# russellgeum/Digging-into-Self-Supervised-Monocular-Depth-Estimation

Hardware: AMD Instinct MI355X
Metric: images/sec training, KITTI 192x640 batch 12/GPU (higher is better)
Workload: dtype f32; 1 GPU; configs[1]: kitti_eigen_zhou-shaped 192x640, batch 12/GPU, ResNet18 depth + separate ResNet18 pose, frame_ids [0,-1,1], 4 scales, automask, Adam, fp32; global_batch=12, parallelism=dp1

## Files before the change

digging-into-self-supervised-monocular-depth-estimation_amd/csrc/norm_nhwc.hip:

```cpp
#include "nhwc_common.hpp"

namespace mdx {
namespace nhwc {

constexpr int STATS_FWD_BLOCKS = 256;
constexpr int STATS_BWD_BLOCKS_F32 = 256, STATS_BWD_BLOCKS_BF16 = 384;
constexpr int STATS_MAX_BLOCKS = 384;
constexpr int APPLY_MAX_BLOCKS = 4096;
constexpr int STATS_ITERS = 8, APPLY_ITERS = 4;
static inline int stats_bwd_blocks(int dtype) { return dtype == 0 ? STATS_BWD_BLOCKS_F32 : STATS_BWD_BLOCKS_BF16; }

template <typename T>
__global__ __launch_bounds__(NB) void bn_nhwc_fwd_stats_kernel(const T *__restrict__ x, int M, int C, int CVB, int PL, int RB,
                                                               float *__restrict__ part)
{
    constexpr int N = VecN<T>::N;
    __shared__ float lds[2 * NB * N];
    const Pos p = position<N>(M, C, CVB, PL, RB);
    float a[N], q[N];
#pragma unroll
    for (int j = 0; j < N; ++j) a[j] = q[j] = 0.f;
    if (p.active) {
        const T *px = x + (size_t)p.g * M * C + (size_t)p.cv * N;
        auto acc = [&](const Vec<T, N> &v) {
// ... 137 lines not shown
    for (; r + 3 * PL < p.r1; r += 4 * PL) {
        const size_t o0 = (size_t)r * C, o1 = (size_t)(r + PL) * C, o2 = (size_t)(r + 2 * PL) * C, o3 = (size_t)(r + 3 * PL) * C;
        const Vec<T, N> v0 = load_vec<T, N>(px + o0), v1 = load_vec<T, N>(px + o1), v2 = load_vec<T, N>(px + o2), v3 = load_vec<T, N>(px + o3);
        Vec<T, N> r0 = {}, r1 = {}, r2 = {}, r3 = {};
        if (pr) { r0 = load_vec<T, N>(pr + o0); r1 = load_vec<T, N>(pr + o1); r2 = load_vec<T, N>(pr + o2); r3 = load_vec<T, N>(pr + o3); }
        apply(v0, r0, o0); apply(v1, r1, o1); apply(v2, r2, o2); apply(v3, r3, o3);
    }
    for (; r < p.r1; r += PL) {
        const size_t o = (size_t)r * C;
        Vec<T, N> rv = {};
        if (pr) rv = load_vec<T, N>(pr + o);
        apply(load_vec<T, N>(px + o), rv, o);
    }
}

template <typename T, bool MASKX>
__global__ __launch_bounds__(NB) void bn_nhwc_bwd_stats_kernel(const T *__restrict__ dy, const T *__restrict__ dy2,
                                                               const T *__restrict__ y, const T *__restrict__ x,
                                                               const float *__restrict__ gamma, const float *__restrict__ beta,
                                                               const float *__restrict__ save_mean,
                                                               const float *__restrict__ save_invstd, int M, int C, int CVB, int PL,
                                                               int RB, int relu, float *__restrict__ part)
{
    constexpr int N = VecN<T>::N;
    __shared__ float lds[2 * NB * N];
    const Pos p = position<N>(M, C, CVB, PL, RB);
    float a[N], q[N];
#pragma unroll
    for (int j = 0; j < N; ++j) a[j] = q[j] = 0.f;
    if (p.active) {
        float mean[N], invstd[N], scale[N], shift[N];
#pragma unroll
        for (int j = 0; j < N; ++j) {
            mean[j] = save_mean[(size_t)p.g * C + p.cv * N + j];
            invstd[j] = save_invstd[(size_t)p.g * C + p.cv * N + j];
            scale[j] = shift[j] = 0.f;
            if (MASKX) {
                scale[j] = gamma[p.cv * N + j] * invstd[j];
                shift[j] = beta[p.cv * N + j] - mean[j] * scale[j];
            }
        }
        const size_t base = (size_t)p.g * M * C + (size_t)p.cv * N;
        const T *pd = dy + base, *pd2 = dy2 ? dy2 + base : nullptr, *py = MASKX ? nullptr : y + base, *px = x + base;
        auto acc = [&](const Vec<T, N> &vd, const Vec<T, N> &vd2, const Vec<T, N> &vy, const Vec<T, N> &vx) {
#pragma unroll
            for (int j = 0; j < N; ++j) {
                float d = to_float(vd.v[j]);
                if (pd2) d += to_float(vd2.v[j]);
                const float yv = !MASKX ? to_float(vy.v[j]) : to_float(from_float<T>(__builtin_fmaf(to_float(vx.v[j]), scale[j], shift[j])));
                const float dz = (relu && !(yv > 0.f)) ? 0.f : d;
                a[j] += dz;
                q[j] = __builtin_fmaf(dz, (to_float(vx.v[j]) - mean[j]) * invstd[j], q[j]);
            }
        };
        int r = p.r0 + p.pl;
        for (; r + PL < p.r1; r += 2 * PL) {
            const size_t o0 = (size_t)r * C, o1 = (size_t)(r + PL) * C;
            const Vec<T, N> d0 = load_vec<T, N>(pd + o0), d1 = load_vec<T, N>(pd + o1);
            Vec<T, N> y0 = {}, y1 = {};
            if (!MASKX) { y0 = load_vec<T, N>(py + o0); y1 = load_vec<T, N>(py + o1); }
            const Vec<T, N> x0 = load_vec<T, N>(px + o0), x1 = load_vec<T, N>(px + o1);
            Vec<T, N> e0 = {}, e1 = {};
            if (pd2) { e0 = load_vec<T, N>(pd2 + o0); e1 = load_vec<T, N>(pd2 + o1); }
            acc(d0, e0, y0, x0);
            acc(d1, e1, y1, x1);
        }
        for (; r < p.r1; r += PL) {
            const size_t o = (size_t)r * C;
            Vec<T, N> e = {}, yv = {};
            if (pd2) e = load_vec<T, N>(pd2 + o);
            if (!MASKX) yv = load_vec<T, N>(py + o);
            acc(load_vec<T, N>(pd + o), e, yv, load_vec<T, N>(px + o));
        }
    }
    block_partials<N>(a, q, lds, CVB, PL, C, part + ((size_t)p.g * gridDim.x + blockIdx.x) * 2 * C);
}

template <typename T, bool MASKX>
__global__ __launch_bounds__(NB) void bn_nhwc_bwd_apply_kernel(const T *__restrict__ dy, const T *__restrict__ dy2,
                                                               const T *__restrict__ y, const T *__restrict__ x,
                                                               const float *__restrict__ gamma, const float *__restrict__ beta,
                                                               const float *__restrict__ save_mean,
                                                               const float *__restrict__ save_invstd,
                                                               const float *__restrict__ totals, int M, int C, int CVB, int PL,
                                                               int RB, int relu, T *__restrict__ dx, T *__restrict__ dres)
{
    constexpr int N = VecN<T>::N;
    const Pos p = position<N>(M, C, CVB, PL, RB);
    if (!p.active) return;
    float mean[N], invstd[N], k0[N], mdz[N], mdzx[N], shift[N];
#pragma unroll
    for (int j = 0; j < N; ++j) {
        const int c = p.cv * N + j;
        mean[j] = save_mean[(size_t)p.g * C + c];
        invstd[j] = save_invstd[(size_t)p.g * C + c];
        k0[j] = gamma[c] * invstd[j];
        shift[j] = MASKX ? beta[c] - mean[j] * k0[j] : 0.f;
        mdz[j] = totals[((size_t)p.g * 2 + 0) * C + c];
        mdzx[j] = totals[((size_t)p.g * 2 + 1) * C + c];
    }
    const size_t base = (size_t)p.g * M * C + (size_t)p.cv * N;
    const T *pd = dy + base, *pd2 = dy2 ? dy2 + base : nullptr, *py = MASKX ? nullptr : y + base, *px = x + base;
    T *ox = dx + base;
    T *orr = dres ? dres + base : nullptr;
    auto apply = [&](const Vec<T, N> &vd, const Vec<T, N> &vd2, const Vec<T, N> &vy, const Vec<T, N> &vx, size_t off) {
        Vec<T, N> wx, wr;
#pragma unroll
        for (int j = 0; j < N; ++j) {
            float d = to_float(vd.v[j]);
            if (pd2) d += to_float(vd2.v[j]);
            const float yv = !MASKX ? to_float(vy.v[j]) : to_float(from_float<T>(__builtin_fmaf(to_float(vx.v[j]), k0[j], shift[j])));
            const float dz = (relu && !(yv > 0.f)) ? 0.f : d;
            const float xh = (to_float(vx.v[j]) - mean[j]) * invstd[j];
            wx.v[j] = from_float<T>(k0[j] * (dz - mdz[j] - xh * mdzx[j]));
            wr.v[j] = from_float<T>(dz);
        }
        store_vec<T, N>(ox + off, wx);
        if (orr) store_vec<T, N>(orr + off, wr);
    };
    int r = p.r0 + p.pl;
    for (; r + PL < p.r1; r += 2 * PL) {
        const size_t o0 = (size_t)r * C, o1 = (size_t)(r + PL) * C;
        const Vec<T, N> d0 = load_vec<T, N>(pd + o0), d1 = load_vec<T, N>(pd + o1);
        Vec<T, N> y0 = {}, y1 = {};
        if (!MASKX) { y0 = load_vec<T, N>(py + o0); y1 = load_vec<T, N>(py + o1); }
        const Vec<T, N> x0 = load_vec<T, N>(px + o0), x1 = load_vec<T, N>(px + o1);
        Vec<T, N> e0 = {}, e1 = {};
        if (pd2) { e0 = load_vec<T, N>(pd2 + o0); e1 = load_vec<T, N>(pd2 + o1); }
        apply(d0, e0, y0, x0, o0);
        apply(d1, e1, y1, x1, o1);
    }
    for (; r < p.r1; r += PL) {
        const size_t o = (size_t)r * C;
        Vec<T, N> e = {}, yv = {};
        if (pd2) e = load_vec<T, N>(pd2 + o);
        if (!MASKX) yv = load_vec<T, N>(py + o);
        apply(load_vec<T, N>(pd + o), e, yv, load_vec<T, N>(px + o), o);
    }
}

static inline int vec_elems(int dtype) { return dtype == 0 ? 4 : 8; }

}
}

using namespace mdx;
using namespace mdx::nhwc;

MDX_EXPORT size_t mdx_bn_nhwc_workspace_bytes(int B, int C, int H, int W, int groups, int dtype)
{
    if (B <= 0 || C <= 0 || H <= 0 || W <= 0 || groups <= 0 || (dtype != 0 && dtype != 1)) return 0;
    const Rows g = make_rows((long long)B * H * W, C, vec_elems(dtype), STATS_MAX_BLOCKS, STATS_ITERS);
// ... 52 lines not shown
    if (bad) return bad;
    if (!aligned(dy, 16) || (y && !aligned(y, 16)) || !aligned(x, 16) || !aligned(dx, 16) || (dy2 && !aligned(dy2, 16)) ||
        (dres && !aligned(dres, 16)))
        return MDX_ERR_MISALIGNED;
    if (workspace_bytes < mdx_bn_nhwc_workspace_bytes(B, C, H, W, groups, dtype)) return MDX_ERR_WORKSPACE;
    const int M = B * H * W, N = vec_elems(dtype);
    const Rows gs = make_rows(M, C, N, stats_bwd_blocks(dtype), STATS_ITERS), ga = make_rows(M, C, N, APPLY_MAX_BLOCKS, APPLY_ITERS);
    float *part = (float *)workspace;
    float *totals = part + (size_t)groups * gs.nblk * 2 * C;
    hipStream_t st = (hipStream_t)stream;
    const dim3 grid_s(gs.nblk, gs.t.ny, groups), grid_a(ga.nblk, ga.t.ny, groups), block(NB);
    const bool maskx = !y;
#define MDX_BN_BWD(KERNEL, T, MX, ...) hipLaunchKernelGGL((KERNEL<T, MX>), __VA_ARGS__)
    if (dtype == 0 && maskx)
        MDX_BN_BWD(bn_nhwc_bwd_stats_kernel, float, true, grid_s, block, 0, st, (const float *)dy, (const float *)dy2, (const float *)y,
                   (const float *)x, gamma, beta, save_mean, save_invstd, M, C, gs.t.CVB, gs.t.PL, gs.RB, relu, part);
    else if (dtype == 0)
        MDX_BN_BWD(bn_nhwc_bwd_stats_kernel, float, false, grid_s, block, 0, st, (const float *)dy, (const float *)dy2, (const float *)y,
                   (const float *)x, gamma, beta, save_mean, save_invstd, M, C, gs.t.CVB, gs.t.PL, gs.RB, relu, part);
    else if (maskx)
        MDX_BN_BWD(bn_nhwc_bwd_stats_kernel, bf16, true, grid_s, block, 0, st, (const bf16 *)dy, (const bf16 *)dy2, (const bf16 *)y,
                   (const bf16 *)x, gamma, beta, save_mean, save_invstd, M, C, gs.t.CVB, gs.t.PL, gs.RB, relu, part);
    else
        MDX_BN_BWD(bn_nhwc_bwd_stats_kernel, bf16, false, grid_s, block, 0, st, (const bf16 *)dy, (const bf16 *)dy2, (const bf16 *)y,
                   (const bf16 *)x, gamma, beta, save_mean, save_invstd, M, C, gs.t.CVB, gs.t.PL, gs.RB, relu, part);
    hipLaunchKernelGGL(bn_nhwc_bwd_finalize_kernel, dim3((C + FC - 1) / FC), dim3(FC * FS), 0, st, part, gs.nblk, C, groups, (double)M, totals,
                       dgamma, dbeta);
    if (dtype == 0 && maskx)
        MDX_BN_BWD(bn_nhwc_bwd_apply_kernel, float, true, grid_a, block, 0, st, (const float *)dy, (const float *)dy2, (const float *)y,
                   (const float *)x, gamma, beta, save_mean, save_invstd, totals, M, C, ga.t.CVB, ga.t.PL, ga.RB, relu, (float *)dx, (float *)dres);
    else if (dtype == 0)
        MDX_BN_BWD(bn_nhwc_bwd_apply_kernel, float, false, grid_a, block, 0, st, (const float *)dy, (const float *)dy2, (const float *)y,
                   (const float *)x, gamma, beta, save_mean, save_invstd, totals, M, C, ga.t.CVB, ga.t.PL, ga.RB, relu, (float *)dx, (float *)dres);
    else if (maskx)
        MDX_BN_BWD(bn_nhwc_bwd_apply_kernel, bf16, true, grid_a, block, 0, st, (const bf16 *)dy, (const bf16 *)dy2, (const bf16 *)y,
                   (const bf16 *)x, gamma, beta, save_mean, save_invstd, totals, M, C, ga.t.CVB, ga.t.PL, ga.RB, relu, (bf16 *)dx, (bf16 *)dres);
    else
        MDX_BN_BWD(bn_nhwc_bwd_apply_kernel, bf16, false, grid_a, block, 0, st, (const bf16 *)dy, (const bf16 *)dy2, (const bf16 *)y,
                   (const bf16 *)x, gamma, beta, save_mean, save_invstd, totals, M, C, ga.t.CVB, ga.t.PL, ga.RB, relu, (bf16 *)dx, (bf16 *)dres);
#undef MDX_BN_BWD
    return check_launch();
}
```

digging-into-self-supervised-monocular-depth-estimation_amd/mdx/functional.py:

```python
import ctypes as C

import torch

from . import _lib
from ._lib import api, ptr, stream


def _f32c(t):
    return t.contiguous().float() if (t.dtype != torch.float32 or not t.is_contiguous()) else t


def _ws(nbytes, device):
    return torch.empty(max(int(nbytes), 8) // 8 + 1, dtype=torch.float64, device=device)


class _ComposeProjection(torch.autograd.Function):
    @staticmethod
    def forward(ctx, K, T):
        K, T = _f32c(K), _f32c(T)
        B = K.shape[0]
        P = torch.empty(B, 3, 4, device=K.device, dtype=torch.float32)
        api.mdx_compose_projection(ptr(K), ptr(T), B, ptr(P), stream())
        ctx.save_for_backward(K, T)
        return P
# ... 976 lines not shown
            nws = api.mdx_bn_workspace_bytes(Bg, Cc, H, W)
            ws = torch.empty(nws // 4 + 1, device=x.device, dtype=torch.float32)
            api.mdx_bn_act_bwd(
                ptr(dy, x.dtype), ptr(y, x.dtype), ptr(x, x.dtype), ptr(weight), ptr(save_mean), ptr(save_invstd),
                ptr(dx, x.dtype), ptr(dres, x.dtype) if has_res else None, ptr(dgamma), ptr(dbeta), Bg, Cc, H, W, groups,
                int(relu), code, ptr(ws), nws, stream())
        return (dx, dres, dgamma, dbeta) + (None,) * 7


def bn_act(x, weight, bias, running_mean, running_var, eps=1e-5, momentum=0.1, residual=None, relu=True, groups=1,
           fork=False):
    return _BnAct.apply(x, residual, weight, bias, running_mean, running_var, float(eps), float(momentum), bool(relu),
                        int(groups), bool(fork))


def bn_act_infer(x, weight, bias, running_mean, running_var, eps=1e-5, residual=None, relu=True, fork=False):
    code = _glue_dtype(x, "bn_act_infer")
    B, Cc, H, W = x.shape
    cl = is_channels_last(x) and _nhwc_ok(x.dtype, Cc)
    x = _as(x, cl)
    if residual is not None:
        if residual.shape != x.shape or residual.dtype != x.dtype:
            raise _lib.MdxError("bn_act_infer: residual %s %s does not match x %s %s"
                                % (tuple(residual.shape), residual.dtype, tuple(x.shape), x.dtype))
        residual = _as(residual, cl)
    y = torch.empty_like(x)
    fn = api.mdx_bn_act_nhwc_infer if cl else api.mdx_bn_act_infer
    fn(ptr(x, x.dtype, cl=cl), ptr(residual, x.dtype, cl=cl) if residual is not None else None, ptr(_f32c(weight)),
       ptr(_f32c(bias)), ptr(_f32c(running_mean)), ptr(_f32c(running_var)), ptr(y, x.dtype, cl=cl), B, Cc, H, W, float(eps),
       int(bool(relu)), code, stream())
# ... 78 lines not shown
```

digging-into-self-supervised-monocular-depth-estimation_amd/model_layer/depth_encoder.py:

```python
import os
import warnings

import numpy as np
import torch
import torch.nn as nn
import torch.nn.functional as TF



class BatchNorm2d(nn.BatchNorm2d):

    fused_min_elements = 0
    fused_eval = True
    _batch_groups = 1

    @staticmethod
    def batch_groups(groups, network):
        import contextlib

        @contextlib.contextmanager
        def scope():
            mods = [m for m in network.modules() if isinstance(m, BatchNorm2d)]
            prev = [m.__dict__.get("_batch_groups") for m in mods]
            for m in mods:
# ... 21 lines not shown
        return self._norm(x)

    def _norm(self, x):
        if self.training:
            self._pending_batches += 1
        return TF.batch_norm(x, self.running_mean, self.running_var, self.weight, self.bias, self.training,
                             self.momentum, self.eps)

    def act(self, x, residual=None, relu=True, fork=False):
        if not self.training and self._eval_fused(x, residual):
            from mdx import functional as F
            if residual is not None and residual.dtype != x.dtype:
                residual = residual.to(x.dtype)
            return F.bn_act_infer(x, self.weight, self.bias, self.running_mean, self.running_var, self.eps,
                                  residual=residual, relu=relu, fork=fork)
        fused = (self.training and x.is_cuda and self.track_running_stats and self.momentum is not None
                 and self.affine and x.dtype in (torch.float32, torch.bfloat16) and x.dim() == 4
                 and torch.is_grad_enabled() and x.shape[0] % self._batch_groups == 0
                 and x.shape[0] * x.shape[2] * x.shape[3] >= self.fused_min_elements
                 and (x.shape[0] // self._batch_groups) * ((x.shape[2] * x.shape[3] + 8191) // 8192) <= 65535)
        if not fused:
            out = self(x)
            if residual is not None:
                out = out + residual
            out = TF.relu(out) if relu else out
            return (out, out) if fork else out
        from mdx import functional as F
        self._pending_batches += self._batch_groups
        if residual is not None and residual.dtype != x.dtype:
            residual = residual.to(x.dtype)
        return F.bn_act(x, self.weight, self.bias, self.running_mean, self.running_var, self.eps, self.momentum,
                        residual=residual, relu=relu, groups=self._batch_groups, fork=fork)

    def _eval_fused(self, x, residual):
        if not (self.fused_eval and x.is_cuda and x.dtype in (torch.float32, torch.bfloat16) and x.dim() == 4
                and self.track_running_stats and self.affine and self.running_mean is not None):
            return False
        return not torch.is_grad_enabled() or not any(
            t is not None and t.requires_grad for t in (x, residual, self.weight, self.bias))

    def _flush_counter(self):
        if self._pending_batches and self.num_batches_tracked is not None:
            self.num_batches_tracked += self._pending_batches
        self._pending_batches = 0

    def _save_to_state_dict(self, destination, prefix, keep_vars):
        self._flush_counter()
        super()._save_to_state_dict(destination, prefix, keep_vars)

    def _load_from_state_dict(self, *args, **kwargs):
        self._pending_batches = 0
        super()._load_from_state_dict(*args, **kwargs)

def _pair(x):
    return x if isinstance(x, tuple) else (x, x)


class BasicBlock(nn.Module):
    expansion = 1
    fork_output = True

    def __init__(self, inplanes, planes, stride=1, downsample=None):
        super().__init__()
        self.conv1 = nn.Conv2d(inplanes, planes, 3, stride, 1, bias=False)
        self.bn1 = BatchNorm2d(planes)
        self.relu = nn.ReLU(inplace=True)
        self.conv2 = nn.Conv2d(planes, planes, 3, 1, 1, bias=False)
# ... 94 lines not shown
        super().__init__()
        self.num_ch_enc = np.array([64, 64, 128, 256, 512])
        if num_layers not in _CFG:
            raise ValueError("{} is not a valid number of resnet layers".format(num_layers))
        if num_input_images > 1:
            self.encoder = resnet_multiimage_input(num_layers, pretrained, num_input_images)
        else:
            block, layers = _CFG[num_layers]
            self.encoder = ResNet(block, layers)
            if pretrained:
                _load_pretrained(self.encoder, num_layers, 1)
        if num_layers > 34:
            self.num_ch_enc[1:] *= 4

    fused_input = True

    def _normalised_input(self, input_image):
        from mdx import functional as F
        from mdx.layout import weight_layout
        stack = input_image if isinstance(input_image, F.FrameStack) else None
        if stack is None and torch.is_tensor(input_image) and input_image.dim() == 4 and input_image.shape[1] == 3:
            stack = F.FrameStack([[input_image]])
        if (self.fused_input and stack is not None and stack.ok() and weight_layout(self.encoder.conv1)
                and stack.blocks[0][0].numel() * len(stack.blocks) * len(stack.blocks[0]) < (1 << 31)):
            dt = torch.get_autocast_gpu_dtype() if torch.is_autocast_enabled() else torch.float32
            if dt in (torch.float32, torch.bfloat16):
                return F.encoder_input(stack, 0.45, 0.225, dt)
        if isinstance(input_image, F.FrameStack):
            input_image = input_image.tensor()
        return (input_image - 0.45) / 0.225

    def forward(self, input_image):
        from mdx.layout import to_layout, weight_layout
        self.features = []
        x = self._normalised_input(input_image)
        stem, stem_b = _pair(self.encoder.bn1.act(self.encoder.conv1(x), fork=BasicBlock.fork_output))
        self.features.append(stem)
        if (stem.is_cuda and stem.dtype in (torch.float32, torch.bfloat16)
                and stem.shape[0] * stem.shape[1] <= 65535):
            from mdx import functional as F
            x = F.maxpool3s2(stem_b, fork=BasicBlock.fork_output)
        else:
            x = self.encoder.maxpool(stem_b)
        for layer in (self.encoder.layer1, self.encoder.layer2, self.encoder.layer3, self.encoder.layer4):
            x = _pair(layer(to_layout(x, weight_layout(layer)) if x[0].is_cuda else x))
            self.features.append(x[0])
        return self.features
```

digging-into-self-supervised-monocular-depth-estimation_amd/model_tool/loader.py:

```python
import os

import torch
from torch.utils.data import DataLoader
from torch.utils.data.distributed import DistributedSampler

from model_layer import *
from model_loss import *
from .synthetic import SyntheticKITTI


def _opt(opt, name, default):
    return getattr(opt, name, default)


def collate_step_keys(samples):
    from torch.utils.data import default_collate
    from .processor import step_reads
    return default_collate([{k: v for k, v in s.items() if step_reads(k)} for s in samples])


def collate_raw_step_keys(samples):
    from model_loader.kitti import collate_raw
    from .processor import step_reads
    return collate_raw(samples, step_reads)
# ... 55 lines not shown
                          drop_last=True, pin_memory=str(self.device).startswith("cuda"),
                          collate_fn=(collate_raw_step_keys if getattr(dataset, "gpu_prep", False) or getattr(dataset, "raw", False)
                                      else collate_step_keys if _opt(opt, "collate_step_keys", False) else None),
                          persistent_workers=workers > 0, prefetch_factor=(_opt(opt, "prefetch_factor", 4) if workers > 0 else None))

    def set_model(self):
        opt = self.opt
        self.model["encoder"] = ResnetEncoder(num_layers=opt.num_layers, pretrained=opt.weight_init)
        self.model["decoder"] = DepthDecoder(num_ch_enc=self.model["encoder"].num_ch_enc, scales=opt.scales)
        if opt.pose_type == "posecnn":
            self.model["pose_decoder"] = PoseCNN(num_input_frames=self.num_pose_frames)
        elif opt.pose_type == "shared":
            self.model["pose_decoder"] = PoseDecoder(self.model["encoder"].num_ch_enc, self.num_pose_frames)
        elif opt.pose_type == "separate":
            self.model["pose_encoder"] = ResnetEncoder(opt.num_layers, opt.weight_init, self.num_pose_frames)
            self.model["pose_decoder"] = PoseDecoder(self.model["pose_encoder"].num_ch_enc, num_input_features=1,
                                                     num_frames_to_predict_for=2)
        self.inv_projection = {0: Depth2PointCloud(opt.batch, opt.height, opt.width).to(self.device)}
        self.for_projection = {0: PointCloud2Pixel(opt.batch, opt.height, opt.width).to(self.device)}
        for key in self.model:
            self.model[key] = self.model[key].to(self.device)
        from mdx.layout import apply_plan
        plan = _opt(opt, "channels_last", "auto")
        if plan == "auto" and not str(self.device).startswith("cuda"):
            plan = "none"
        self.channels_last_stages = apply_plan(self.model, plan)
        for key in self.model:
            m = self.model[key]
            for name, p in m.named_parameters():
                if name.startswith("encoder.fc."):
# ... 34 lines not shown
```

include/mdx.h:

```cpp
#ifndef MDX_H
#define MDX_H

#include <stddef.h>
#include <stdint.h>

#ifdef __cplusplus
extern "C" {
#endif

#define MDX_VERSION 510
#define MDX_MAX_SRC 4
#define MDX_MAX_SCALES 4

typedef enum mdx_status {
    MDX_OK = 0,
    MDX_ERR_BAD_SHAPE = -1,
    MDX_ERR_NULL_POINTER = -2,
    MDX_ERR_WORKSPACE = -3,
    MDX_ERR_LAUNCH = -4,
    MDX_ERR_UNSUPPORTED = -5,
    MDX_ERR_MISALIGNED = -6
} mdx_status;

#define MDX_FLAG_AUTOMASK 1u
// ... 182 lines not shown
                     const float *run_var, void *y, int B, int C, int H, int W, float eps, int relu, int dtype,
                     void *stream);
int mdx_bn_act_nhwc_infer(const void *x, const void *res, const float *gamma, const float *beta, const float *run_mean,
                          const float *run_var, void *y, int B, int C, int H, int W, float eps, int relu, int dtype,
                          void *stream);

size_t mdx_bn_nhwc_workspace_bytes(int B, int C, int H, int W, int groups, int dtype);
int mdx_bn_act_nhwc_fwd(const void *x, const void *res, const float *gamma, const float *beta, float *run_mean,
                        float *run_var, void *y, float *save_mean, float *save_invstd, int B, int C, int H, int W,
                        int groups, float eps, float momentum, int relu, int dtype, void *workspace,
                        size_t workspace_bytes, void *stream);
int mdx_bn_act_nhwc_bwd(const void *dy, const void *dy2, const void *y, const void *x, const float *gamma,
                        const float *beta, const float *save_mean, const float *save_invstd, void *dx, void *dres, float *dgamma,
                        float *dbeta, int B, int C, int H, int W, int groups, int relu, int dtype, void *workspace,
                        size_t workspace_bytes, void *stream);
size_t mdx_bias_act_nhwc_workspace_bytes(int B, int C, int H, int W, int dtype);
int mdx_bias_act_nhwc_fwd(const void *x, const float *bias, void *y, int B, int C, int H, int W, int relu, int dtype, void *stream);
int mdx_bias_act_nhwc_bwd(const void *dy, const void *y, void *dx, float *dbias, int B, int C, int H, int W, int relu, int dtype,
                          void *workspace, size_t workspace_bytes, void *stream);
int mdx_mean_bias_nhwc_fwd(const void *x, const float *bias, float *out, int B, int C, int H, int W, float scale, int dtype,
                           void *stream);
int mdx_mean_bias_nhwc_bwd(const float *gout, void *dx, float *dbias, int B, int C, int H, int W, float scale, int dtype,
                           void *stream);

int mdx_encoder_input_nhwc(const float *const *src, int blocks, int groups, int n, int H, int W, float mean, float inv_std,
                           void *out, int dtype, void *stream);

size_t mdx_thin_conv3x3_wgrad_workspace_bytes(int B, int Cin, int Cout, int h, int w);
int mdx_thin_conv3x3_wgrad(const float *x, const float *gy, float *gweight, int64_t s_o, int64_t s_c, int64_t s_y, int64_t s_x, int B,
                           int Cin, int Cout, int h, int w, void *workspace, size_t workspace_bytes, void *stream);
// ... 66 lines not shown
```

Before: 824.7 images/s.

## Fuse stem BN+ReLU with 3x3 stride-2 maxpool forward and backward

```diff
diff --git a/digging-into-self-supervised-monocular-depth-estimation_amd/csrc/norm_nhwc.hip b/digging-into-self-supervised-monocular-depth-estimation_amd/csrc/norm_nhwc.hip
--- a/digging-into-self-supervised-monocular-depth-estimation_amd/csrc/norm_nhwc.hip
+++ b/digging-into-self-supervised-monocular-depth-estimation_amd/csrc/norm_nhwc.hip
@@ -175,13 +175,141 @@
     }
 }
 
-template <typename T, bool MASKX>
+template <typename T, bool WRITEY>
+__global__ __launch_bounds__(NB) void bn_pool_nhwc_fwd_apply_kernel(const T *__restrict__ x, const float *__restrict__ gamma,
+                                                                    const float *__restrict__ beta,
+                                                                    const float *__restrict__ save_mean,
+                                                                    const float *__restrict__ save_invstd, T *__restrict__ y,
+                                                                    T *__restrict__ pooled, uint8_t *__restrict__ arg, int B, int C,
+                                                                    int H, int W, int Ho, int Wo, int CVB, int XL)
+{
+    constexpr int N = VecN<T>::N;
+    const int xl = threadIdx.x / CVB, xo = blockIdx.y * XL + xl;
+    const int c0 = (blockIdx.z * CVB + threadIdx.x % CVB) * N;
+    if (xl >= XL || xo >= Wo || c0 >= C) return;
+    const int b = blockIdx.x / Ho, yo = blockIdx.x - b * Ho, g = b / B;
+    float scale[N], shift[N];
+#pragma unroll
+    for (int j = 0; j < N; ++j) {
+        const int c = c0 + j;
+        scale[j] = gamma[c] * save_invstd[(size_t)g * C + c];
+        shift[j] = beta[c] - save_mean[(size_t)g * C + c] * scale[j];
+    }
+    const size_t img = (size_t)b * H * W * C + c0;
+    Vec<T, N> tap[9];
+    bool ok[9];
+#pragma unroll
+    for (int k = 0; k < 9; ++k) {
+        const int yy = 2 * yo - 1 + k / 3, xx = 2 * xo - 1 + k % 3;
+        ok[k] = yy >= 0 && yy < H && xx >= 0 && xx < W;
+        tap[k] = load_vec<T, N>(x + img + ((size_t)(ok[k] ? yy : 0) * W + (ok[k] ? xx : 0)) * C);
+    }
+#pragma unroll
+    for (int k = 0; k < 9; ++k)
+#pragma unroll
+        for (int j = 0; j < N; ++j) {
+            const float f = __builtin_fmaf(to_float(tap[k].v[j]), scale[j], shift[j]);
+            tap[k].v[j] = from_float<T>(f < 0.f ? 0.f : f);
+        }
+    if (WRITEY) {
+#pragma unroll
+        for (int k = 4; k < 9; ++k) {
+            if (k == 6 || !ok[k]) continue;
+            const int yy = 2 * yo - 1 + k / 3, xx = 2 * xo - 1 + k % 3;
+            store_vec<T, N>(y + img + ((size_t)yy * W + xx) * C, tap[k]);
+        }
+    }
+    Vec<T, N> o;
+    Vec<uint8_t, N> a;
+#pragma unroll
+    for (int j = 0; j < N; ++j) {
+        float best = -INFINITY;
+        int bi = -1;
+#pragma unroll
+        for (int k = 0; k < 9; ++k) {
+            if (!ok[k]) continue;
+            const float v = to_float(tap[k].v[j]);
+            if (bi < 0) bi = k;
+            if (v > best || v != v) { best = v; bi = k; }
+        }
+        o.v[j] = from_float<T>(best);
+        a.v[j] = (uint8_t)bi;
+    }
+    const size_t off = ((size_t)blockIdx.x * Wo + xo) * C + c0;
+    store_vec<T, N>(pooled + off, o);
+    store_vec<uint8_t, N>(arg + off, a);
+}
+
+template <typename T> struct PoolSrc {
+    const T *gpool, *gpool2;
+    const uint8_t *arg;
+    int B, H, W, Ho, Wo;
+    int sb, sy, sx;
+};
+struct Pix { int b, y, x; };
+__device__ __forceinline__ Pix pix_of(int r, int H, int W)
+{
+    Pix q;
+    q.b = r / (H * W);
+    const int rem = r - q.b * H * W;
+    q.y = rem / W;
+    q.x = rem - q.y * W;
+    return q;
+}
+template <typename T> __device__ __forceinline__ void pix_step(Pix &q, const PoolSrc<T> &s)
+{
+    q.x += s.sx; q.y += s.sy; q.b += s.sb;
+    if (q.x >= s.W) { q.x -= s.W; ++q.y; }
+    if (q.y >= s.H) { q.y -= s.H; ++q.b; }
+}
+template <typename T, int N>
+__device__ __forceinline__ void pool_gather(const PoolSrc<T> &s, int C, int img, const Pix &q, int c0, float (&g)[N])
+{
+    const int yo0 = q.y >> 1, xo0 = q.x >> 1;
+    const int ny = (q.y & 1) ? 2 : 1, nx = (q.x & 1) ? 2 : 1;
+    const size_t base = (size_t)img * s.Ho * s.Wo * C + c0;
+#pragma unroll
+    for (int j = 0; j < N; ++j) g[j] = 0.f;
+    Vec<T, N> gv[2][2], gw[2][2] = {};
+    Vec<uint8_t, N> av[2][2];
+    bool ok[2][2];
+#pragma unroll
+    for (int i = 0; i < 2; ++i)
+#pragma unroll
+        for (int k = 0; k < 2; ++k) {
+            const int yo = yo0 + i, xo = xo0 + k;
+            ok[i][k] = i < ny && k < nx && yo < s.Ho && xo < s.Wo;
+            gv[i][k] = Vec<T, N>{};
+            av[i][k] = Vec<uint8_t, N>{};
+            if (ok[i][k]) {
+                const size_t off = base + ((size_t)yo * s.Wo + xo) * C;
+                gv[i][k] = load_vec<T, N>(s.gpool + off);
+                if (s.gpool2) gw[i][k] = load_vec<T, N>(s.gpool2 + off);
+                av[i][k] = load_vec<uint8_t, N>(s.arg + off);
+            }
+        }
+#pragma unroll
+    for (int i = 0; i < 2; ++i)
+#pragma unroll
+        for (int k = 0; k < 2; ++k) {
+            if (!ok[i][k]) continue;
+            const int tapi = (q.y - 2 * (yo0 + i) + 1) * 3 + (q.x - 2 * (xo0 + k) + 1);
+#pragma unroll
+            for (int j = 0; j < N; ++j)
+                if ((int)av[i][k].v[j] == tapi)
+                    g[j] += s.gpool2 ? to_float(gv[i][k].v[j]) + to_float(gw[i][k].v[j]) : to_float(gv[i][k].v[j]);
+        }
+#pragma unroll
+    for (int j = 0; j < N; ++j) g[j] = to_float(from_float<T>(g[j]));
+}
+
+template <typename T, bool MASKX, bool POOL = false>
 __global__ __launch_bounds__(NB) void bn_nhwc_bwd_stats_kernel(const T *__restrict__ dy, const T *__restrict__ dy2,
                                                                const T *__restrict__ y, const T *__restrict__ x,
                                                                const float *__restrict__ gamma, const float *__restrict__ beta,
                                                                const float *__restrict__ save_mean,
                                                                const float *__restrict__ save_invstd, int M, int C, int CVB, int PL,
-                                                               int RB, int relu, float *__restrict__ part)
+                                                               int RB, int relu, float *__restrict__ part, const PoolSrc<T> ps)
 {
     constexpr int N = VecN<T>::N;
     __shared__ float lds[2 * NB * N];
@@ -202,12 +330,18 @@
             }
         }
         const size_t base = (size_t)p.g * M * C + (size_t)p.cv * N;
-        const T *pd = dy + base, *pd2 = dy2 ? dy2 + base : nullptr, *py = MASKX ? nullptr : y + base, *px = x + base;
-        auto acc = [&](const Vec<T, N> &vd, const Vec<T, N> &vd2, const Vec<T, N> &vy, const Vec<T, N> &vx) {
+        const T *pd = (!POOL || dy) ? dy + base : nullptr, *pd2 = (!POOL && dy2) ? dy2 + base : nullptr;
+        const T *py = MASKX ? nullptr : y + base, *px = x + base;
+        auto acc = [&](const Vec<T, N> &vd, const Vec<T, N> &vd2, const float (&gp)[N], const Vec<T, N> &vy, const Vec<T, N> &vx) {
 #pragma unroll
             for (int j = 0; j < N; ++j) {
-                float d = to_float(vd.v[j]);
-                if (pd2) d += to_float(vd2.v[j]);
+                float d;
+                if (POOL) {
+                    d = pd ? to_float(vd.v[j]) + gp[j] : gp[j];
+                } else {
+                    d = to_float(vd.v[j]);
+                    if (pd2) d += to_float(vd2.v[j]);
+                }
                 const float yv = !MASKX ? to_float(vy.v[j]) : to_float(from_float<T>(__builtin_fmaf(to_float(vx.v[j]), scale[j], shift[j])));
                 const float dz = (relu && !(yv > 0.f)) ? 0.f : d;
                 a[j] += dz;
@@ -215,36 +349,54 @@
             }
         };
         int r = p.r0 + p.pl;
+        Pix pix = {};
+        if (POOL) pix = pix_of(r, ps.H, ps.W);
+        const int c0 = p.cv * N;
         for (; r + PL < p.r1; r += 2 * PL) {
             const size_t o0 = (size_t)r * C, o1 = (size_t)(r + PL) * C;
-            const Vec<T, N> d0 = load_vec<T, N>(pd + o0), d1 = load_vec<T, N>(pd + o1);
+            Vec<T, N> d0 = {}, d1 = {};
+            if (!POOL || pd) { d0 = load_vec<T, N>(pd + o0); d1 = load_vec<T, N>(pd + o1); }
             Vec<T, N> y0 = {}, y1 = {};
             if (!MASKX) { y0 = load_vec<T, N>(py + o0); y1 = load_vec<T, N>(py + o1); }
             const Vec<T, N> x0 = load_vec<T, N>(px + o0), x1 = load_vec<T, N>(px + o1);
             Vec<T, N> e0 = {}, e1 = {};
             if (pd2) { e0 = load_vec<T, N>(pd2 + o0); e1 = load_vec<T, N>(pd2 + o1); }
-            acc(d0, e0, y0, x0);
-            acc(d1, e1, y1, x1);
+            float g0[N] = {}, g1[N] = {};
+            if (POOL) {
+                pool_gather<T, N>(ps, C, p.g * ps.B + pix.b, pix, c0, g0);
+                pix_step(pix, ps);
+                pool_gather<T, N>(ps, C, p.g * ps.B + pix.b, pix, c0, g1);
+                pix_step(pix, ps);
+            }
+            acc(d0, e0, g0, y0, x0);
+            acc(d1, e1, g1, y1, x1);
         }
         for (; r < p.r1; r += PL) {
             const size_t o = (size_t)r * C;
-            Vec<T, N> e = {}, yv = {};
+            Vec<T, N> e = {}, yv = {}, d = {};
             if (pd2) e = load_vec<T, N>(pd2 + o);
             if (!MASKX) yv = load_vec<T, N>(py + o);
-            acc(load_vec<T, N>(pd + o), e, yv, load_vec<T, N>(px + o));
+            if (!POOL || pd) d = load_vec<T, N>(pd + o);
+            float g0[N] = {};
+            if (POOL) {
+                pool_gather<T, N>(ps, C, p.g * ps.B + pix.b, pix, c0, g0);
+                pix_step(pix, ps);
+            }
+            acc(d, e, g0, yv, load_vec<T, N>(px + o));
         }
     }
     block_partials<N>(a, q, lds, CVB, PL, C, part + ((size_t)p.g * gridDim.x + blockIdx.x) * 2 * C);
 }
 
-template <typename T, bool MASKX>
+template <typename T, bool MASKX, bool POOL = false>
 __global__ __launch_bounds__(NB) void bn_nhwc_bwd_apply_kernel(const T *__restrict__ dy, const T *__restrict__ dy2,
                                                                const T *__restrict__ y, const T *__restrict__ x,
                                                                const float *__restrict__ gamma, const float *__restrict__ beta,
                                                                const float *__restrict__ save_mean,
                                                                const float *__restrict__ save_invstd,
                                                                const float *__restrict__ totals, int M, int C, int CVB, int PL,
-                                                               int RB, int relu, T *__restrict__ dx, T *__restrict__ dres)
+                                                               int RB, int relu, T *__restrict__ dx, T *__restrict__ dres,
+                                                               const PoolSrc<T> ps)
 {
     constexpr int N = VecN<T>::N;
     const Pos p = position<N>(M, C, CVB, PL, RB);
@@ -261,15 +413,21 @@
         mdzx[j] = totals[((size_t)p.g * 2 + 1) * C + c];
     }
     const size_t base = (size_t)p.g * M * C + (size_t)p.cv * N;
-    const T *pd = dy + base, *pd2 = dy2 ? dy2 + base : nullptr, *py = MASKX ? nullptr : y + base, *px = x + base;
+    const T *pd = (!POOL || dy) ? dy + base : nullptr, *pd2 = (!POOL && dy2) ? dy2 + base : nullptr;
+    const T *py = MASKX ? nullptr : y + base, *px = x + base;
     T *ox = dx + base;
-    T *orr = dres ? dres + base : nullptr;
-    auto apply = [&](const Vec<T, N> &vd, const Vec<T, N> &vd2, const Vec<T, N> &vy, const Vec<T, N> &vx, size_t off) {
+    T *orr = (!POOL && dres) ? dres + base : nullptr;
+    auto apply = [&](const Vec<T, N> &vd, const Vec<T, N> &vd2, const float (&gp)[N], const Vec<T, N> &vy, const Vec<T, N> &vx, size_t off) {
         Vec<T, N> wx, wr;
 #pragma unroll
         for (int j = 0; j < N; ++j) {
-            float d = to_float(vd.v[j]);
-            if (pd2) d += to_float(vd2.v[j]);
+            float d;
+            if (POOL) {
+                d = pd ? to_float(vd.v[j]) + gp[j] : gp[j];
+            } else {
+                d = to_float(vd.v[j]);
+                if (pd2) d += to_float(vd2.v[j]);
+            }
             const float yv = !MASKX ? to_float(vy.v[j]) : to_float(from_float<T>(__builtin_fmaf(to_float(vx.v[j]), k0[j], shift[j])));
             const float dz = (relu && !(yv > 0.f)) ? 0.f : d;
             const float xh = (to_float(vx.v[j]) - mean[j]) * invstd[j];
@@ -280,23 +438,40 @@
         if (orr) store_vec<T, N>(orr + off, wr);
     };
     int r = p.r0 + p.pl;
+    Pix pix = {};
+    if (POOL) pix = pix_of(r, ps.H, ps.W);
+    const int c0 = p.cv * N;
     for (; r + PL < p.r1; r += 2 * PL) {
         const size_t o0 = (size_t)r * C, o1 = (size_t)(r + PL) * C;
-        const Vec<T, N> d0 = load_vec<T, N>(pd + o0), d1 = load_vec<T, N>(pd + o1);
+        Vec<T, N> d0 = {}, d1 = {};
+        if (!POOL || pd) { d0 = load_vec<T, N>(pd + o0); d1 = load_vec<T, N>(pd + o1); }
         Vec<T, N> y0 = {}, y1 = {};
         if (!MASKX) { y0 = load_vec<T, N>(py + o0); y1 = load_vec<T, N>(py + o1); }
         const Vec<T, N> x0 = load_vec<T, N>(px + o0), x1 = load_vec<T, N>(px + o1);
         Vec<T, N> e0 = {}, e1 = {};
         if (pd2) { e0 = load_vec<T, N>(pd2 + o0); e1 = load_vec<T, N>(pd2 + o1); }
-        apply(d0, e0, y0, x0, o0);
-        apply(d1, e1, y1, x1, o1);
+        float g0[N] = {}, g1[N] = {};
+        if (POOL) {
+            pool_gather<T, N>(ps, C, p.g * ps.B + pix.b, pix, c0, g0);
+            pix_step(pix, ps);
+            pool_gather<T, N>(ps, C, p.g * ps.B + pix.b, pix, c0, g1);
+            pix_step(pix, ps);
+        }
+        apply(d0, e0, g0, y0, x0, o0);
+        apply(d1, e1, g1, y1, x1, o1);
     }
     for (; r < p.r1; r += PL) {
         const size_t o = (size_t)r * C;
-        Vec<T, N> e = {}, yv = {};
+        Vec<T, N> e = {}, yv = {}, d = {};
         if (pd2) e = load_vec<T, N>(pd2 + o);
         if (!MASKX) yv = load_vec<T, N>(py + o);
-        apply(load_vec<T, N>(pd + o), e, yv, load_vec<T, N>(px + o), o);
+        if (!POOL || pd) d = load_vec<T, N>(pd + o);
+        float g0[N] = {};
+        if (POOL) {
+            pool_gather<T, N>(ps, C, p.g * ps.B + pix.b, pix, c0, g0);
+            pix_step(pix, ps);
+        }
+        apply(d, e, g0, yv, load_vec<T, N>(px + o), o);
     }
 }
 
@@ -379,30 +554,112 @@
 #define MDX_BN_BWD(KERNEL, T, MX, ...) hipLaunchKernelGGL((KERNEL<T, MX>), __VA_ARGS__)
     if (dtype == 0 && maskx)
         MDX_BN_BWD(bn_nhwc_bwd_stats_kernel, float, true, grid_s, block, 0, st, (const float *)dy, (const float *)dy2, (const float *)y,
-                   (const float *)x, gamma, beta, save_mean, save_invstd, M, C, gs.t.CVB, gs.t.PL, gs.RB, relu, part);
+                   (const float *)x, gamma, beta, save_mean, save_invstd, M, C, gs.t.CVB, gs.t.PL, gs.RB, relu, part, PoolSrc<float>{});
     else if (dtype == 0)
         MDX_BN_BWD(bn_nhwc_bwd_stats_kernel, float, false, grid_s, block, 0, st, (const float *)dy, (const float *)dy2, (const float *)y,
-                   (const float *)x, gamma, beta, save_mean, save_invstd, M, C, gs.t.CVB, gs.t.PL, gs.RB, relu, part);
+                   (const float *)x, gamma, beta, save_mean, save_invstd, M, C, gs.t.CVB, gs.t.PL, gs.RB, relu, part, PoolSrc<float>{});
     else if (maskx)
         MDX_BN_BWD(bn_nhwc_bwd_stats_kernel, bf16, true, grid_s, block, 0, st, (const bf16 *)dy, (const bf16 *)dy2, (const bf16 *)y,
-                   (const bf16 *)x, gamma, beta, save_mean, save_invstd, M, C, gs.t.CVB, gs.t.PL, gs.RB, relu, part);
+                   (const bf16 *)x, gamma, beta, save_mean, save_invstd, M, C, gs.t.CVB, gs.t.PL, gs.RB, relu, part, PoolSrc<bf16>{});
     else
         MDX_BN_BWD(bn_nhwc_bwd_stats_kernel, bf16, false, grid_s, block, 0, st, (const bf16 *)dy, (const bf16 *)dy2, (const bf16 *)y,
-                   (const bf16 *)x, gamma, beta, save_mean, save_invstd, M, C, gs.t.CVB, gs.t.PL, gs.RB, relu, part);
+                   (const bf16 *)x, gamma, beta, save_mean, save_invstd, M, C, gs.t.CVB, gs.t.PL, gs.RB, relu, part, PoolSrc<bf16>{});
     hipLaunchKernelGGL(bn_nhwc_bwd_finalize_kernel, dim3((C + FC - 1) / FC), dim3(FC * FS), 0, st, part, gs.nblk, C, groups, (double)M, totals,
                        dgamma, dbeta);
     if (dtype == 0 && maskx)
         MDX_BN_BWD(bn_nhwc_bwd_apply_kernel, float, true, grid_a, block, 0, st, (const float *)dy, (const float *)dy2, (const float *)y,
-                   (const float *)x, gamma, beta, save_mean, save_invstd, totals, M, C, ga.t.CVB, ga.t.PL, ga.RB, relu, (float *)dx, (float *)dres);
+                   (const float *)x, gamma, beta, save_mean, save_invstd, totals, M, C, ga.t.CVB, ga.t.PL, ga.RB, relu, (float *)dx, (float *)dres, PoolSrc<float>{});
     else if (dtype == 0)
         MDX_BN_BWD(bn_nhwc_bwd_apply_kernel, float, false, grid_a, block, 0, st, (const float *)dy, (const float *)dy2, (const float *)y,
-                   (const float *)x, gamma, beta, save_mean, save_invstd, totals, M, C, ga.t.CVB, ga.t.PL, ga.RB, relu, (float *)dx, (float *)dres);
+                   (const float *)x, gamma, beta, save_mean, save_invstd, totals, M, C, ga.t.CVB, ga.t.PL, ga.RB, relu, (float *)dx, (float *)dres, PoolSrc<float>{});
     else if (maskx)
         MDX_BN_BWD(bn_nhwc_bwd_apply_kernel, bf16, true, grid_a, block, 0, st, (const bf16 *)dy, (const bf16 *)dy2, (const bf16 *)y,
-                   (const bf16 *)x, gamma, beta, save_mean, save_invstd, totals, M, C, ga.t.CVB, ga.t.PL, ga.RB, relu, (bf16 *)dx, (bf16 *)dres);
+                   (const bf16 *)x, gamma, beta, save_mean, save_invstd, totals, M, C, ga.t.CVB, ga.t.PL, ga.RB, relu, (bf16 *)dx, (bf16 *)dres, PoolSrc<bf16>{});
     else
         MDX_BN_BWD(bn_nhwc_bwd_apply_kernel, bf16, false, grid_a, block, 0, st, (const bf16 *)dy, (const bf16 *)dy2, (const bf16 *)y,
-                   (const bf16 *)x, gamma, beta, save_mean, save_invstd, totals, M, C, ga.t.CVB, ga.t.PL, ga.RB, relu, (bf16 *)dx, (bf16 *)dres);
+                   (const bf16 *)x, gamma, beta, save_mean, save_invstd, totals, M, C, ga.t.CVB, ga.t.PL, ga.RB, relu, (bf16 *)dx, (bf16 *)dres, PoolSrc<bf16>{});
 #undef MDX_BN_BWD
     return check_launch();
 }
+
+static int pool_args_ok(int B, int C, int H, int W, int groups, int dtype)
+{
+    const int bad = nhwc_args_ok(B, C, H, W, groups, dtype);
+    if (bad) return bad;
+    if ((long long)groups * B * H >= (1ll << 31)) return MDX_ERR_BAD_SHAPE;
+    const Tile t = make_tile(C, vec_elems(dtype));
+    if (((W - 1) / 2 + 1 + t.PL - 1) / t.PL > 65535) return MDX_ERR_BAD_SHAPE;
+    return MDX_OK;
+}
+
+MDX_EXPORT int mdx_bn_act_pool_nhwc_fwd(const void *x, const float *gamma, const float *beta, float *run_mean, float *run_var, void *y,
+                                        void *pooled, uint8_t *arg, float *save_mean, float *save_invstd, int B, int C, int H, int W,
+                                        int groups, float eps, float momentum, int dtype, void *workspace, size_t workspace_bytes,
+                                        void *stream)
+{
+    if (!x || !gamma || !beta || !pooled || !arg || !save_mean || !save_invstd || !workspace) return MDX_ERR_NULL_POINTER;
+    if ((run_mean == nullptr) != (run_var == nullptr)) return MDX_ERR_NULL_POINTER;
+    const int bad = pool_args_ok(B, C, H, W, groups, dtype);
+    if (bad) return bad;
+    if (!y && dtype != 0) return MDX_ERR_NULL_POINTER;
+    if (!aligned(x, 16) || (y && !aligned(y, 16)) || !aligned(pooled, 16) || !aligned(arg, 8)) return MDX_ERR_MISALIGNED;
+    if (workspace_bytes < mdx_bn_nhwc_workspace_bytes(B, C, H, W, groups, dtype)) return MDX_ERR_WORKSPACE;
+    const int M = B * H * W, N = vec_elems(dtype), Ho = (H - 1) / 2 + 1, Wo = (W - 1) / 2 + 1;
+    const Rows gs = make_rows(M, C, N, STATS_FWD_BLOCKS, STATS_ITERS);
+    float *part = (float *)workspace;
+    hipStream_t st = (hipStream_t)stream;
+    const dim3 grid_s(gs.nblk, gs.t.ny, groups), grid_p(groups * B * Ho, (Wo + gs.t.PL - 1) / gs.t.PL, gs.t.ny), block(NB);
+    if (dtype == 0)
+        hipLaunchKernelGGL((bn_nhwc_fwd_stats_kernel<float>), grid_s, block, 0, st, (const float *)x, M, C, gs.t.CVB, gs.t.PL, gs.RB, part);
+    else
+        hipLaunchKernelGGL((bn_nhwc_fwd_stats_kernel<bf16>), grid_s, block, 0, st, (const bf16 *)x, M, C, gs.t.CVB, gs.t.PL, gs.RB, part);
+    hipLaunchKernelGGL(bn_nhwc_fwd_finalize_kernel, dim3((C + FC - 1) / FC), dim3(FC * FS), 0, st, part, gs.nblk, C, groups, (double)M,
+                       eps, momentum, save_mean, save_invstd, run_mean, run_var);
+#define MDX_BN_POOL_FWD(T, WY)                                                                                                        \
+    hipLaunchKernelGGL((bn_pool_nhwc_fwd_apply_kernel<T, WY>), grid_p, block, 0, st, (const T *)x, gamma, beta, save_mean, save_invstd, \
+                       (T *)y, (T *)pooled, arg, B, C, H, W, Ho, Wo, gs.t.CVB, gs.t.PL)
+    if (dtype == 0 && y) MDX_BN_POOL_FWD(float, true);
+    else if (dtype == 0) MDX_BN_POOL_FWD(float, false);
+    else MDX_BN_POOL_FWD(bf16, true);
+#undef MDX_BN_POOL_FWD
+    return check_launch();
+}
+
+MDX_EXPORT int mdx_bn_act_pool_nhwc_bwd(const void *dy, const void *gpool, const void *gpool2, const uint8_t *arg, const void *y,
+                                        const void *x, const float *gamma, const float *beta, const float *save_mean,
+                                        const float *save_invstd, void *dx, float *dgamma, float *dbeta, int B, int C, int H, int W,
+                                        int groups, int dtype, void *workspace, size_t workspace_bytes, void *stream)
+{
+    if (!gpool || !arg || !x || !gamma || !save_mean || !save_invstd || !dx || !dgamma || !dbeta || !workspace)
+        return MDX_ERR_NULL_POINTER;
+    const int bad = pool_args_ok(B, C, H, W, groups, dtype);
+    if (bad) return bad;
+    if (dtype == 0 ? (y != nullptr || !beta) : !y) return MDX_ERR_NULL_POINTER;
+    if ((dy && !aligned(dy, 16)) || !aligned(gpool, 16) || (gpool2 && !aligned(gpool2, 16)) || !aligned(arg, 8) ||
+        (y && !aligned(y, 16)) || !aligned(x, 16) || !aligned(dx, 16))
+        return MDX_ERR_MISALIGNED;
+    if (workspace_bytes < mdx_bn_nhwc_workspace_bytes(B, C, H, W, groups, dtype)) return MDX_ERR_WORKSPACE;
+    const int M = B * H * W, N = vec_elems(dtype);
+    const Rows gs = make_rows(M, C, N, stats_bwd_blocks(dtype), STATS_ITERS), ga = make_rows(M, C, N, APPLY_MAX_BLOCKS, APPLY_ITERS);
+    float *part = (float *)workspace;
+    float *totals = part + (size_t)groups * gs.nblk * 2 * C;
+    hipStream_t st = (hipStream_t)stream;
+    const dim3 grid_s(gs.nblk, gs.t.ny, groups), grid_a(ga.nblk, ga.t.ny, groups), block(NB);
+    const int PL = gs.t.PL;
+    const int Ho = (H - 1) / 2 + 1, Wo = (W - 1) / 2 + 1;
+#define MDX_BN_POOL_BWD(T, MX)                                                                                                         \
+    do {                                                                                                                               \
+        const PoolSrc<T> ps = {(const T *)gpool, (const T *)gpool2, arg, B, H, W, Ho, Wo, PL / (H * W), PL % (H * W) / W, PL % W};     \
+        hipLaunchKernelGGL((bn_nhwc_bwd_stats_kernel<T, MX, true>), grid_s, block, 0, st, (const T *)dy, (const T *)nullptr,           \
+                           (const T *)y, (const T *)x, gamma, beta, save_mean, save_invstd, M, C, gs.t.CVB, PL, gs.RB, 1, part, ps);   \
+        hipLaunchKernelGGL(bn_nhwc_bwd_finalize_kernel, dim3((C + FC - 1) / FC), dim3(FC * FS), 0, st, part, gs.nblk, C, groups,       \
+                           (double)M, totals, dgamma, dbeta);                                                                          \
+        hipLaunchKernelGGL((bn_nhwc_bwd_apply_kernel<T, MX, true>), grid_a, block, 0, st, (const T *)dy, (const T *)nullptr,           \
+                           (const T *)y, (const T *)x, gamma, beta, save_mean, save_invstd, totals, M, C, ga.t.CVB, PL, ga.RB, 1,      \
+                           (T *)dx, (T *)nullptr, ps);                                                                                 \
+    } while (0)
+    if (dtype == 0) MDX_BN_POOL_BWD(float, true);
+    else MDX_BN_POOL_BWD(bf16, false);
+#undef MDX_BN_POOL_BWD
+    return check_launch();
+}
diff --git a/digging-into-self-supervised-monocular-depth-estimation_amd/mdx/functional.py b/digging-into-self-supervised-monocular-depth-estimation_amd/mdx/functional.py
--- a/digging-into-self-supervised-monocular-depth-estimation_amd/mdx/functional.py
+++ b/digging-into-self-supervised-monocular-depth-estimation_amd/mdx/functional.py
@@ -1014,6 +1014,79 @@
                         int(groups), bool(fork))
 
 
+class _BnActPool(torch.autograd.Function):
+
+    @staticmethod
+    def forward(ctx, x, weight, bias, running_mean, running_var, eps, momentum, groups, want_y, fork):
+        code = _glue_dtype(x, "bn_act_pool")
+        B, Cc, H, W = x.shape
+        if B % groups:
+            raise _lib.MdxError("bn_act_pool: batch %d is not divisible into %d groups" % (B, groups))
+        if not (x.is_contiguous(memory_format=_CL) and _nhwc_ok(x.dtype, Cc)):
+            raise _lib.MdxError("bn_act_pool takes channels-last maps of whole 16-byte channel vectors, got %s %s strides %s"
+                                % (x.dtype, tuple(x.shape), x.stride()))
+        if not want_y and x.dtype != torch.float32:
+            raise _lib.MdxError("bn_act_pool: want_y=False is a float32 form (the bfloat16 backward reads its mask from y)")
+        weight, bias = _f32c(weight), _f32c(bias)
+        Ho, Wo = (H - 1) // 2 + 1, (W - 1) // 2 + 1
+        y = torch.empty_like(x) if want_y else None
+        pooled = torch.empty(B, Cc, Ho, Wo, device=x.device, dtype=x.dtype, memory_format=_CL)
+        arg = torch.empty(B, Cc, Ho, Wo, device=x.device, dtype=torch.uint8, memory_format=_CL)
+        save_mean = torch.empty(groups, Cc, device=x.device, dtype=torch.float32)
+        save_invstd = torch.empty(groups, Cc, device=x.device, dtype=torch.float32)
+        Bg = B // groups
+        nws = api.mdx_bn_nhwc_workspace_bytes(Bg, Cc, H, W, groups, code)
+        ws = torch.empty(nws // 4 + 1, device=x.device, dtype=torch.float32)
+        api.mdx_bn_act_pool_nhwc_fwd(
+            ptr(x, x.dtype, cl=True), ptr(weight), ptr(bias), ptr(running_mean) if running_mean is not None else None,
+            ptr(running_var) if running_var is not None else None, ptr(y, x.dtype, cl=True) if want_y else None,
+            ptr(pooled, x.dtype, cl=True), ptr(arg, torch.uint8, cl=True), ptr(save_mean), ptr(save_invstd), Bg, Cc, H, W,
+            groups, eps, momentum, code, ptr(ws), nws, stream())
+        mask_from_x = x.dtype == torch.float32
+        ctx.save_for_backward(x, bias if mask_from_x else y, weight, save_mean, save_invstd, arg)
+        ctx.meta = (groups, mask_from_x)
+        ctx.mark_non_differentiable(*[t for t in (running_mean, running_var) if t is not None])
+        ctx.set_materialize_grads(False)
+        return (y, pooled, pooled.view_as(pooled)) if fork else (y, pooled)
+
+    @staticmethod
+    def backward(ctx, dy, gpool, gpool2=None):
+        x, y, weight, save_mean, save_invstd, arg = ctx.saved_tensors
+        groups, mask_from_x = ctx.meta
+        bias = None
+        if mask_from_x:
+            y, bias = None, y
+        none = (None,) * 10
+        (dy, _), (gpool, gpool2) = _two_grads(dy, None, x.dtype, True, True), _two_grads(gpool, gpool2, x.dtype, True, True)
+        if dy is None and gpool is None:
+            return none
+        B, Cc, H, W = x.shape
+        Bg = B // groups
+        code = _DTYPE_CODE[x.dtype]
+        dx = torch.empty_like(x)
+        dgamma = torch.empty(Cc, device=x.device, dtype=torch.float32)
+        dbeta = torch.empty(Cc, device=x.device, dtype=torch.float32)
+        nws = api.mdx_bn_nhwc_workspace_bytes(Bg, Cc, H, W, groups, code)
+        ws = torch.empty(nws // 4 + 1, device=x.device, dtype=torch.float32)
+        opt = lambda t, dt=x.dtype: ptr(t, dt, cl=True) if t is not None else None
+        if gpool is None:
+            api.mdx_bn_act_nhwc_bwd(
+                opt(dy), None, opt(y), ptr(x, x.dtype, cl=True), ptr(weight), ptr(bias) if bias is not None else None,
+                ptr(save_mean), ptr(save_invstd), ptr(dx, x.dtype, cl=True), None, ptr(dgamma), ptr(dbeta), Bg, Cc, H, W,
+                groups, 1, code, ptr(ws), nws, stream())
+        else:
+            api.mdx_bn_act_pool_nhwc_bwd(
+                opt(dy), opt(gpool), opt(gpool2), ptr(arg, torch.uint8, cl=True), opt(y), ptr(x, x.dtype, cl=True),
+                ptr(weight), ptr(bias) if bias is not None else None, ptr(save_mean), ptr(save_invstd),
+                ptr(dx, x.dtype, cl=True), ptr(dgamma), ptr(dbeta), Bg, Cc, H, W, groups, code, ptr(ws), nws, stream())
+        return (dx, dgamma, dbeta) + (None,) * 7
+
+
+def bn_act_pool(x, weight, bias, running_mean, running_var, eps=1e-5, momentum=0.1, groups=1, want_y=True, fork=False):
+    return _BnActPool.apply(x, weight, bias, running_mean, running_var, float(eps), float(momentum), int(groups),
+                            bool(want_y), bool(fork))
+
+
 def bn_act_infer(x, weight, bias, running_mean, running_var, eps=1e-5, residual=None, relu=True, fork=False):
     code = _glue_dtype(x, "bn_act_infer")
     B, Cc, H, W = x.shape
diff --git a/digging-into-self-supervised-monocular-depth-estimation_amd/model_layer/depth_encoder.py b/digging-into-self-supervised-monocular-depth-estimation_amd/model_layer/depth_encoder.py
--- a/digging-into-self-supervised-monocular-depth-estimation_amd/model_layer/depth_encoder.py
+++ b/digging-into-self-supervised-monocular-depth-estimation_amd/model_layer/depth_encoder.py
@@ -59,12 +59,7 @@
                 residual = residual.to(x.dtype)
             return F.bn_act_infer(x, self.weight, self.bias, self.running_mean, self.running_var, self.eps,
                                   residual=residual, relu=relu, fork=fork)
-        fused = (self.training and x.is_cuda and self.track_running_stats and self.momentum is not None
-                 and self.affine and x.dtype in (torch.float32, torch.bfloat16) and x.dim() == 4
-                 and torch.is_grad_enabled() and x.shape[0] % self._batch_groups == 0
-                 and x.shape[0] * x.shape[2] * x.shape[3] >= self.fused_min_elements
-                 and (x.shape[0] // self._batch_groups) * ((x.shape[2] * x.shape[3] + 8191) // 8192) <= 65535)
-        if not fused:
+        if not self._train_fused(x):
             out = self(x)
             if residual is not None:
                 out = out + residual
@@ -76,6 +71,25 @@
             residual = residual.to(x.dtype)
         return F.bn_act(x, self.weight, self.bias, self.running_mean, self.running_var, self.eps, self.momentum,
                         residual=residual, relu=relu, groups=self._batch_groups, fork=fork)
+
+    def _train_fused(self, x):
+        return (self.training and x.is_cuda and self.track_running_stats and self.momentum is not None
+                and self.affine and x.dtype in (torch.float32, torch.bfloat16) and x.dim() == 4
+                and torch.is_grad_enabled() and x.shape[0] % self._batch_groups == 0
+                and x.shape[0] * x.shape[2] * x.shape[3] >= self.fused_min_elements
+                and (x.shape[0] // self._batch_groups) * ((x.shape[2] * x.shape[3] + 8191) // 8192) <= 65535)
+
+    def act_pool_ok(self, x, want_y=True):
+        from mdx import functional as F
+        return (type(self).act is _FUSED_ACT and self._train_fused(x) and x.shape[0] * x.shape[1] <= 65535
+                and F.is_channels_last(x) and x.shape[1] % (4 if x.dtype == torch.float32 else 8) == 0
+                and (want_y or x.dtype == torch.float32))
+
+    def act_pool(self, x, want_y=True, fork=False):
+        from mdx import functional as F
+        self._pending_batches += self._batch_groups
+        return F.bn_act_pool(x, self.weight, self.bias, self.running_mean, self.running_var, self.eps, self.momentum,
+                             groups=self._batch_groups, want_y=want_y, fork=fork)
 
     def _eval_fused(self, x, residual):
         if not (self.fused_eval and x.is_cuda and x.dtype in (torch.float32, torch.bfloat16) and x.dim() == 4
@@ -96,6 +110,10 @@
     def _load_from_state_dict(self, *args, **kwargs):
         self._pending_batches = 0
         super()._load_from_state_dict(*args, **kwargs)
+
+
+_FUSED_ACT = BatchNorm2d.act
+
 
 def _pair(x):
     return x if isinstance(x, tuple) else (x, x)
@@ -220,6 +238,8 @@
             self.num_ch_enc[1:] *= 4
 
     fused_input = True
+    fused_stem_pool = os.environ.get("MDX_STEM_POOL", "1") != "0"
+    stem_feature = True
 
     def _normalised_input(self, input_image):
         from mdx import functional as F
@@ -237,10 +257,16 @@
         return (input_image - 0.45) / 0.225
 
     def forward(self, input_image):
-        from mdx.layout import to_layout, weight_layout
         self.features = []
         x = self._normalised_input(input_image)
-        stem, stem_b = _pair(self.encoder.bn1.act(self.encoder.conv1(x), fork=BasicBlock.fork_output))
+        conv = self.encoder.conv1(x)
+        bn1 = self.encoder.bn1
+        want_y = self.stem_feature or conv.dtype != torch.float32
+        if self.fused_stem_pool and isinstance(bn1, BatchNorm2d) and bn1.act_pool_ok(conv, want_y):
+            stem, *x = bn1.act_pool(conv, want_y=want_y, fork=BasicBlock.fork_output)
+            self.features.append(stem if self.stem_feature else None)
+            return self._layers(tuple(x) if len(x) > 1 else x[0])
+        stem, stem_b = _pair(bn1.act(conv, fork=BasicBlock.fork_output))
         self.features.append(stem)
         if (stem.is_cuda and stem.dtype in (torch.float32, torch.bfloat16)
                 and stem.shape[0] * stem.shape[1] <= 65535):
@@ -248,6 +274,10 @@
             x = F.maxpool3s2(stem_b, fork=BasicBlock.fork_output)
         else:
             x = self.encoder.maxpool(stem_b)
+        return self._layers(x)
+
+    def _layers(self, x):
+        from mdx.layout import to_layout, weight_layout
         for layer in (self.encoder.layer1, self.encoder.layer2, self.encoder.layer3, self.encoder.layer4):
             x = _pair(layer(to_layout(x, weight_layout(layer)) if x[0].is_cuda else x))
             self.features.append(x[0])
diff --git a/digging-into-self-supervised-monocular-depth-estimation_amd/model_tool/loader.py b/digging-into-self-supervised-monocular-depth-estimation_amd/model_tool/loader.py
--- a/digging-into-self-supervised-monocular-depth-estimation_amd/model_tool/loader.py
+++ b/digging-into-self-supervised-monocular-depth-estimation_amd/model_tool/loader.py
@@ -93,6 +93,7 @@
             self.model["pose_decoder"] = PoseDecoder(self.model["encoder"].num_ch_enc, self.num_pose_frames)
         elif opt.pose_type == "separate":
             self.model["pose_encoder"] = ResnetEncoder(opt.num_layers, opt.weight_init, self.num_pose_frames)
+            self.model["pose_encoder"].stem_feature = False
             self.model["pose_decoder"] = PoseDecoder(self.model["pose_encoder"].num_ch_enc, num_input_features=1,
                                                      num_frames_to_predict_for=2)
         self.inv_projection = {0: Depth2PointCloud(opt.batch, opt.height, opt.width).to(self.device)}
diff --git a/include/mdx.h b/include/mdx.h
--- a/include/mdx.h
+++ b/include/mdx.h
@@ -220,6 +220,14 @@
                         const float *beta, const float *save_mean, const float *save_invstd, void *dx, void *dres, float *dgamma,
                         float *dbeta, int B, int C, int H, int W, int groups, int relu, int dtype, void *workspace,
                         size_t workspace_bytes, void *stream);
+int mdx_bn_act_pool_nhwc_fwd(const void *x, const float *gamma, const float *beta, float *run_mean, float *run_var, void *y,
+                             void *pooled, uint8_t *arg, float *save_mean, float *save_invstd, int B, int C, int H, int W,
+                             int groups, float eps, float momentum, int dtype, void *workspace, size_t workspace_bytes,
+                             void *stream);
+int mdx_bn_act_pool_nhwc_bwd(const void *dy, const void *gpool, const void *gpool2, const uint8_t *arg, const void *y,
+                             const void *x, const float *gamma, const float *beta, const float *save_mean,
+                             const float *save_invstd, void *dx, float *dgamma, float *dbeta, int B, int C, int H, int W,
+                             int groups, int dtype, void *workspace, size_t workspace_bytes, void *stream);
 size_t mdx_bias_act_nhwc_workspace_bytes(int B, int C, int H, int W, int dtype);
 int mdx_bias_act_nhwc_fwd(const void *x, const float *bias, void *y, int B, int C, int H, int W, int relu, int dtype, void *stream);
 int mdx_bias_act_nhwc_bwd(const void *dy, const void *y, void *dx, float *dbias, int B, int C, int H, int W, int relu, int dtype,
```

Result: no change. 829.3 images/s (median of 6 runs) (+0.6%).
